# yoshihikosuzuki/ClassPro

Measured on AMD Instinct MI355X. Metric: Mbases/s classified (k=40, 40x HiFi) at 1/2/4/8 MI355X vs CPU -T16, higher is better.
Workload: dtype u16/f64

## Files before the change

### classpro_amd/csrc/capi.hip

```cpp
#include <hip/hip_runtime.h>
#include <stdio.h>
#include <stdlib.h>
#include <string.h>
#include <string>
#include <mutex>
#include <vector>
#include <chrono>
#include <thread>
#include <type_traits>
#include <time.h>
#include "cp_host_setup.h"
#include "kernels.hip"

static thread_local std::string g_err;
static int set_err(int code, const std::string &msg) { g_err = msg; return code; }

#define HIPCHK(call)                                                                       \
  do { hipError_t e_ = (call);                                                             \
       if (e_ != hipSuccess)                                                               \
         return set_err(CP_EHIP,std::string(#call)+": "+hipGetErrorString(e_));            \
     } while (0)
static int launch_status() { HIPCHK(hipGetLastError()); return CP_OK; }

extern "C" const char *cp_last_error(void) { return g_err.c_str(); }
// ... 936 lines not shown
{ if (rlen < 0 || nruns < 0 || K < 1 || (rlen > 0 && !labels) || (nruns > 0 && (!ends || !cls)))
    return set_err(CP_EINVAL,"cp_expand_label_runs: bad argument");
  int pos = K-1 < rlen ? K-1 : rlen;
  memset(labels,'N',(size_t)pos);
  for (int j = 0; j < nruns; j++)
    { const int e = ends[j];
      if (e < pos || e > rlen) return set_err(CP_EINVAL,"cp_expand_label_runs: runs out of order or beyond the read");
      memset(labels+pos,(int)cls[j],(size_t)(e-pos));
      pos = e;
    }
  if (pos != rlen) return set_err(CP_EINVAL,"cp_expand_label_runs: the runs do not cover the read");
  return CP_OK;
}

extern "C" int cp_seq_context(const char *d_seq, const int64_t *d_seq_off, int nreads, int64_t total_bases,
                              uint8_t *d_lctx, uint8_t *d_rctx, void *stream)
{ if (!d_seq || !d_seq_off || !d_lctx || !d_rctx || nreads < 0)
    return set_err(CP_EINVAL,"cp_seq_context: bad argument");
  (void)total_bases;
  if (nreads == 0) return CP_OK;
  hipLaunchKernelGGL(k_seq_context,dim3(nreads),dim3(256),0,(hipStream_t)stream,d_seq,d_seq_off,nreads,d_lctx,d_rctx);
  return launch_status();
}

#ifdef CP_BOUNDS
extern "C" int cp_debug_bounds(unsigned long long *out4)
{ HIPCHK(hipDeviceSynchronize());
  HIPCHK(hipMemcpyFromSymbol(out4,HIP_SYMBOL(g_bounds),sizeof(unsigned long long)*4));
  unsigned long long z[4] = { 0, 0, 0, 0 };
  HIPCHK(hipMemcpyToSymbol(HIP_SYMBOL(g_bounds),z,sizeof(z)));
  return CP_OK;
}
#endif

#if defined(CP_SEED_DEBUG) || defined(CP_SEED_DEBUG_TAKES)
extern "C" int cp_debug_seed_set(int read)
{ HIPCHK(hipMemcpyToSymbol(HIP_SYMBOL(g_seed_dbg_read),&read,sizeof(int))); return CP_OK; }
extern "C" int cp_debug_seed_get(int *out4, int *recs)
{ HIPCHK(hipDeviceSynchronize());
  HIPCHK(hipMemcpyFromSymbol(out4,HIP_SYMBOL(g_seed_dbg_n),16));
  HIPCHK(hipMemcpyFromSymbol(recs,HIP_SYMBOL(g_seed_dbg),8192*16));
  return CP_OK;
}
#endif
#if defined(CP_SEED_PROF) || defined(CP_PROF_WALK)
static int prof_read(unsigned long long *out, const void *sym, size_t n, bool reset = true)
{ static const unsigned long long z[12] = {0};
  HIPCHK(hipMemcpyFromSymbol(out,sym,n*sizeof(unsigned long long)));
  if (reset) HIPCHK(hipMemcpyToSymbol(sym,z,n*sizeof(unsigned long long)));
  return CP_OK;
}
#endif
#ifdef CP_SEED_PROF
extern "C" int cp_debug_seed_prof(unsigned long long *out8)
{ HIPCHK(hipDeviceSynchronize()); return prof_read(out8,HIP_SYMBOL(g_seed_prof),8); }
#endif
extern "C" int cp_debug_task_counts(cp_workspace *ws, int32_t *out, int64_t nreads)
{ if (!ws || !out || nreads < 0 || nreads > ws->nreads || ws->b.fwc.cap < (size_t)nreads*16)
    return set_err(CP_EINVAL,"cp_debug_task_counts: bad arguments");
  HIPCHK(hipDeviceSynchronize());
  if (nreads > 0) HIPCHK(hipMemcpy(out,ws->b.fwc.p,(size_t)nreads*4*sizeof(int32_t),hipMemcpyDeviceToHost));
  return CP_OK;
}
extern "C" int cp_debug_flag_bytes(cp_workspace *ws, int64_t *out2)
{ if (!ws || !out2) return set_err(CP_EINVAL,"cp_debug_flag_bytes: bad arguments");
  HIPCHK(hipDeviceSynchronize());
  const dbuf *arr[2] = { &ws->b.wall, &ws->b.wall_s };
  for (int a = 0; a < 2; a++)
    { std::vector<uint8_t> h(arr[a]->cap);
      if (arr[a]->cap) HIPCHK(hipMemcpy(h.data(),arr[a]->p,arr[a]->cap,hipMemcpyDeviceToHost));
      int64_t n = 0;
      for (uint8_t v : h) n += v != 0;
      out2[a] = n;
    }
  return CP_OK;
}
#ifdef CP_PROF_WALK
extern "C" int cp_debug_live_prof(unsigned long long *out8)
{ HIPCHK(hipDeviceSynchronize()); return prof_read(out8,HIP_SYMBOL(g_live_prof),8); }
extern "C" int cp_debug_emit_prof(unsigned long long *out8)
{ HIPCHK(hipDeviceSynchronize()); return prof_read(out8,HIP_SYMBOL(g_emit_prof),8); }
extern "C" int cp_debug_fw_prof(unsigned long long *out12)
{ HIPCHK(hipDeviceSynchronize()); return prof_read(out12,HIP_SYMBOL(g_fw_prof),12); }
extern "C" int cp_debug_unrel_prof(unsigned long long *out8)
{ HIPCHK(hipDeviceSynchronize()); return prof_read(out8,HIP_SYMBOL(g_unrel_prof),8); }
extern "C" int cp_debug_rel_prof(unsigned long long *out12)
{ HIPCHK(hipDeviceSynchronize()); return prof_read(out12,HIP_SYMBOL(g_rel_prof),12); }
extern "C" int cp_debug_phase_prof(unsigned long long *out36)
{ HIPCHK(hipDeviceSynchronize());
  CHK(prof_read(out36,HIP_SYMBOL(g_phase_max),12));
  CHK(prof_read(out36+12,HIP_SYMBOL(g_phase_sum),12));
  return prof_read(out36+24,HIP_SYMBOL(g_phase_arg),12,false);
}
#endif

#include "kmer_table.hip"

#include "kmer_counts.hip"

#include "kmer_sort.hip"

#include "kmer_lookup.hip"

#include "kmer_hits.hip"

#include "kmer_runs.hip"

#include "kmer_setops.hip"

#include "kmer_cmphist.hip"

#include "kmer_hetpairs.hip"

#include "kmer_unitigs.hip"

#include "kmer_unitig_graph.hip"

#include "kmer_paths.hip"

#include "kmer_prune.hip"

#include "label_tools.hip"
```

### classpro_amd/csrc/kernels.hip

```cpp
#include <hip/hip_runtime.h>
#include <stdint.h>
#include <type_traits>
#include "cp_wall.h"
#include "cp_class.h"
#include "cp_seed.h"

#ifdef CP_BOUNDS
__device__ unsigned long long g_bounds[4];
#endif
#define WAVE 64
#define REL_MAXM 1024
#define UNREL_MAXN 1024
#ifndef REL_SMALL_MAXM
#define REL_SMALL_MAXM 112
#endif
#ifndef UNREL_SMALL_MAXN
#define UNREL_SMALL_MAXN 256
#endif
#define GRP_MAX_PLEN 65535

__device__ __forceinline__ void wave_sync() { __syncthreads(); }
__device__ __forceinline__ void wave_sync_lds()
{ __builtin_amdgcn_fence(__ATOMIC_RELEASE,"wavefront"); __builtin_amdgcn_wave_barrier(); __builtin_amdgcn_fence(__ATOMIC_ACQUIRE,"wavefront"); }

// ... 598 lines not shown
          return true;
        };
      for (int c0 = 0; !done; c0 += WAVE)
        { const int qq = right ? q+1+c0+lane : q-1-c0-lane;
          int pj = 0, fo = 0, fs = 0;
          bool valid = qq >= 0 && qq < F.n;
          if (valid) { pj = F.pos[qq]; valid = right ? (pj < jend) : (pj >= jend); }
          if (valid) { fo = F.fo[qq]; fs = F.fs[qq]; }
          const uint64_t mv = __ballot(valid);
          const uint64_t mw = __ballot(valid && (((fo & CP_W_WALL_O) | (fs & CP_W_WALL_S)) != 0));
          const uint64_t ms = __ballot(valid && (fo & CP_W_WALL_O));
          for (uint64_t t = mw; t; t &= t-1)
            { const int b = __ffsll((long long)t)-1;
              const int jj = __shfl(pj,b), qj = right ? q+1+c0+b : q-1-c0-b;
              if (nx > 0 && !flush_x(jj)) return;
              if (cp_bs_eintvl(ev,0,NS-1,right ? i : jj,right ? jj : i) == -1)
                { const double pe_j = CP_PERR(R,jj,CP_SELF,right ? CP_GAIN : CP_DROP);
                  const double pe = pe_i * pe_j;
                  if (pe >= CP_PE_THRES_FINAL)
                    { if (*midx >= R->ecap) { R->overflow = 1; return; }
                      ev.wave_grow(*midx);
                      if (lane == 0)
                        { cp_eintvl x; x.b = right ? i : jj; x.e = right ? jj : i; x.pe = pe;
                          ev.put(*midx,x);
                          F.fo[q] |= CP_W_PAIRED_M;
                          F.fo[qj] |= CP_W_PAIRED_M;
                        }
                      (*midx)++;
                      if (*midx >= plen) { R->overflow = 8; return; }
                    }
                }
              if ((ms >> b) & 1) { done = true; break; }
            }
          if (mv != ~0ull) break;
        }
      if (nx > 0 && !done && !flush_x(right ? 0x7fffffff : -1)) return;
      if (!done && (right ? plen < jend : jend == 0))
        { const double pe = pe_i * pe_i;
          if (pe >= CP_PE_THRES_FINAL)
            { if (*midx >= R->ecap) { R->overflow = 1; return; }
              ev.wave_grow(*midx);
              if (lane == 0)
                { cp_eintvl x; x.b = right ? i : 0; x.e = right ? plen : i; x.pe = pe;
                  ev.put(*midx,x);
                  F.fo[q] |= CP_W_PAIRED_M;
                }
              (*midx)++;
              if (*midx >= plen) { R->overflow = 8; return; }
            }
        }
      wave_sync();
    }
}

#define CP_PCLS(e,a)   (((uint32_t)(e) << 3) | ((uint32_t)(a) & 7u))
#define CP_PCLS_END(x) ((int)((x) >> 3))
#define CP_PCLS_CLS(x) (((x) & 7u) == 7u ? -1 : (int)((x) & 7u))

struct cp_rrec { int32_t b, e; uint16_t ccb, cce; int32_t idx; double pe; };
static_assert(sizeof(cp_rrec) == 24,"compact reliable-interval record");
struct cp_ivA { int32_t b, e; uint16_t cb, ce, ccb, cce; };
struct cp_ivB { double pe, peo_b, peo_e; };
struct cp_ivC { uint8_t is_rel; int8_t asgn; };
static_assert(sizeof(cp_ivA) == 16 && sizeof(cp_ivB) == 24 && sizeof(cp_ivC) == 2,"interval records as arrays");
struct cp_soa { cp_ivA *a; cp_ivB *b; cp_ivC *c; };
__device__ __forceinline__ void cp_soa_put(const cp_soa &S, int64_t at, const cp_intvl &I)
{ cp_ivA a; a.b = I.b; a.e = I.e; a.cb = I.cb; a.ce = I.ce; a.ccb = I.ccb; a.cce = I.cce;
  cp_ivB b; b.pe = I.pe; b.peo_b = I.peo_b; b.peo_e = I.peo_e;
  cp_ivC c; c.is_rel = I.is_rel; c.asgn = I.asgn;
  S.a[at] = a; S.b[at] = b; S.c[at] = c;
}
__device__ __forceinline__ cp_intvl cp_soa_get(const cp_soa &S, int64_t at)
{ const cp_ivA a = S.a[at]; const cp_ivB b = S.b[at]; const cp_ivC c = S.c[at];
  cp_intvl I;
  memset(&I,0,sizeof(I));
  I.b = a.b; I.e = a.e; I.cb = a.cb; I.ce = a.ce; I.ccb = a.ccb; I.cce = a.cce;
  I.is_rel = c.is_rel; I.asgn = c.asgn; I.pe = b.pe; I.peo_b = b.peo_b; I.peo_e = b.peo_e;
  return I;
}

#ifdef CP_PROF_WALK
__device__ unsigned long long g_phase_max[12], g_phase_sum[12], g_phase_arg[12];
__device__ unsigned long long g_live_prof[8];
__device__ unsigned long long g_unrel_prof[8];
__device__ unsigned long long g_emit_prof[8];
__device__ unsigned long long g_fw_prof[12];
#define EM_LT0() unsigned long long em_t = wall_clock64()
#define EM_LT(k) do { unsigned long long t_ = wall_clock64(); if (lane == 0) atomicAdd(&g_fw_prof[4+(k)],t_-em_t); em_t = wall_clock64(); } while (0)
#define PH_STAMP(k) do { if (lane == 0) { unsigned long long t_ = wall_clock64(); unsigned long long d_ = t_-ph_t; ph_t = t_; \
      atomicAdd(&g_phase_sum[k],d_); unsigned long long o_ = atomicMax(&g_phase_max[k],d_); if (d_ > o_) g_phase_arg[k] = ((unsigned long long)r << 32) | (unsigned)n_c; } } while (0)
#elif defined(CP_STOP_AT)
#define PH_STAMP(k) do { if ((k) == CP_STOP_AT) { PH_STOP_EXTRA; return; } } while (0)
#else
#define PH_STAMP(k) ((void)0)
#endif
#ifndef EM_LT0
#define EM_LT0() ((void)0)
#define EM_LT(k) ((void)0)
#endif
#define PH_STOP_EXTRA

struct task_res { double own_pe, lc_v, hc_pe; int lc_j, hc, pos, kc; };
#define TR_E(hc)     (((hc) >> 3) & 1)
#define TR_WTYPE(hc) (((hc) >> 4) & 1)
static_assert(sizeof(task_res) == 40,"three doubles and four ints, no padding");
static_assert(CP_DROP == 0 && CP_GAIN == 1 && CP_SELF == 0 && CP_OTHERS == 1,"one bit each in task_res::hc");
static_assert(CP_LC_REJECT <= 3,"lc_kind takes two bits of task_res::hc");
struct task_stage { double own_pe, lc_v, hc_pe; int lc_j, hc; };

#define FW_SEQ_WIN    32
#define FW_SEQ_STRIDE 36
struct cp_seq_lwin
  { CP_SEQ_T g; CP_LDS_PTR(const char) w; int lo, len;
    __device__ __forceinline__ char operator[](int p) const
    { const unsigned d = (unsigned)(p-lo); return d < (unsigned)len ? w[d] : g[p]; }
  };
__device__ __forceinline__ int cp_seq_dirword(const cp_seq_lwin &sq, int rlen, int pos, int dir, uint64_t *D)
{ (void)rlen;
  const int d = (dir > 0 ? pos : pos-7)-sq.lo;
  if (d < 0 || d+8 > sq.len) return 0;
  CP_LDS_PTR(const uint32_t) rw = (CP_LDS_PTR(const uint32_t))(sq.w+(d & ~3));
  const uint32_t x0 = rw[0], x1 = rw[1], x2 = rw[2];
  const uint32_t sh = (uint32_t)(d & 3)*8;
  const uint32_t lo = __builtin_amdgcn_alignbit(x1,x0,sh), hi = __builtin_amdgcn_alignbit(x2,x1,sh);
  const uint64_t x = (uint64_t)lo | ((uint64_t)hi << 32);
  *D = dir > 0 ? x : __builtin_bswap64(x);
  return 8;
}
struct __attribute__((packed, aligned(1))) cp_u8x16 { uint32_t v[4]; };
struct __attribute__((packed, aligned(1))) cp_u8x4 { uint32_t v; };
struct cp_seq_rwin
  { CP_SEQ_T g;
    uint64_t wl, wh;
    int lo, len;
    __device__ __forceinline__ char operator[](int p) const
    { const unsigned d = (unsigned)(p-lo);
      if (d < (unsigned)len)
        { const uint64_t x = (d < 8) ? wl : wh;
          return (char)(x >> ((d & 7)*8));
        }
      return g[p];
    }
  };
__device__ __forceinline__ int cp_seq_dirword(const cp_seq_rwin &sq, int rlen, int pos, int dir, uint64_t *D)
{ (void)rlen;
  const int d = (dir > 0 ? pos : pos-7)-sq.lo;
  if (sq.len != 16 || d < 0 || d > 8) return 0;
  const uint64_t x = d == 0 ? sq.wl : d == 8 ? sq.wh : (sq.wl >> (8*d)) | (sq.wh << (64-8*d));
  *D = dir > 0 ? x : __builtin_bswap64(x);
  return 8;
}
struct cp_seq_rsrc { CP_SEQ_T g; };
__device__ __forceinline__ cp_seq_rwin cp_seq_window(const cp_seq_rsrc &src, int pos, int rlen, int dir)
{ cp_seq_rwin sq;
  int lo = dir > 0 ? pos-7 : pos-11;
  if (lo > rlen-16) lo = rlen-16;
  if (lo < 0) lo = 0;
  sq.g = src.g; sq.lo = lo; sq.len = 0; sq.wl = sq.wh = 0;
  if (rlen-lo >= 16)
    { const cp_u8x16 x = *reinterpret_cast<const cp_u8x16 *>(CP_SPAN(src.g,lo,16));
      sq.wl = (uint64_t)x.v[0] | ((uint64_t)x.v[1] << 32);
      sq.wh = (uint64_t)x.v[2] | ((uint64_t)x.v[3] << 32);
      sq.len = 16;
    }
  return sq;
}

// ... 1632 lines not shown
__device__ __forceinline__ void quad_cov_sums(const Rv &rv, const int8_t *asgn, int M, int ld, int cls, int &lsum, int &csum)
{ int ls = 0, cs = 0;
  for (int i = ld; i < M; i += 4)
    if (cls < 0 || asgn[i] == cls)
      { const cp_riv I = rv(i);
        const int l = I.e-I.b;
        ls += l;
        cs += (I.ccb+I.cce)*l/2;
      }
  lsum = quad_isum(ls); csum = quad_isum(cs);
}
__device__ __forceinline__ int quad_count(const int8_t *asgn, int M, int ld, int cls)
{ int n = 0;
  for (int i = ld; i < M; i += 4) n += (asgn[i] == cls);
  return quad_isum(n);
}
__device__ __forceinline__ void quad_first_last(const int8_t *asgn, int M, int ld, int cls, int &first, int &last)
{ int f = M, l = -1;
  for (int i = ld; i < M; i += 4)
    if (asgn[i] == cls) { if (f == M) f = i; l = i; }
  f = quad_imin(f); last = quad_imax(l);
  first = (f == M) ? -1 : f;
}
template <class Rv>
__device__ bool rel_post1_quad(const cp_dev_params *P, const Rv &rv, int M, int F, const int8_t *asgn, int *COV, int ld)
{ const int *G = P->cov;
  if (quad_count(asgn,M,ld,CP_HAPLO)) return false;
  int first_d, last_d;
  quad_first_last(asgn,M,ld,CP_DIPLO,first_d,last_d);
  const int seed = F ? first_d : last_d;
  if (seed < 0) return false;
  int lsum, csum;
  quad_cov_sums(rv,asgn,M,ld,CP_DIPLO,lsum,csum);
  const double mean_dcov = (double)csum/lsum;
  if (!(mean_dcov < G[CP_DIPLO])) return false;
  const cp_riv S = rv(seed);
  COV[CP_HAPLO] = F ? S.ccb : S.cce;
  COV[CP_DIPLO] = (COV[CP_HAPLO]+G[CP_HAPLO]) & 0xffff;
  return true;
}
template <class Rv>
__device__ double rel_post2_quad(const cp_dev_params *P, const Rv &rv, int M, int8_t *asgn, bool rerun, int ld)
{ const int *G = P->cov;
  int lsum, csum;
  if (rerun && quad_count(asgn,M,ld,CP_HAPLO) == 0)
    { quad_cov_sums(rv,asgn,M,ld,CP_DIPLO,lsum,csum);
      const double mean_dcov = (double)csum/lsum;
      if (fabs(mean_dcov-G[CP_HAPLO]) <= fabs(mean_dcov-G[CP_DIPLO]))
        for (int i = ld; i < M; i += 4)
          if (asgn[i] == CP_DIPLO) asgn[i] = CP_HAPLO;
    }
  int n = quad_count(asgn,M,ld,CP_HAPLO);
  if (n == M)
    { quad_cov_sums(rv,asgn,M,ld,-1,lsum,csum);
      const double mean_hcov = (double)csum/lsum;
      if (fabs(mean_hcov-G[CP_HAPLO]) >= fabs(mean_hcov-G[CP_DIPLO]))
        { for (int i = ld; i < M; i += 4) asgn[i] = CP_DIPLO;
          n = 0;
        }
    }
  if (n >= M * 0.7)
    { quad_cov_sums(rv,asgn,M,ld,CP_HAPLO,lsum,csum);
      const double mean_hcov = (double)csum/lsum;
      if (fabs(mean_hcov-G[CP_HAPLO]) >= fabs(mean_hcov-G[CP_DIPLO]))
        for (int i = ld; i < M; i += 4)
          { if (asgn[i] == CP_HAPLO)      asgn[i] = CP_DIPLO;
            else if (asgn[i] == CP_DIPLO) asgn[i] = CP_REPEAT;
          }
    }
  int first_d, last_d, first_h, last_h;
  quad_first_last(asgn,M,ld,CP_DIPLO,first_d,last_d);
  quad_first_last(asgn,M,ld,CP_HAPLO,first_h,last_h);
  if (!(first_d >= 0 && first_h >= 0))
    return 1.;
  return ((double)rv(first_d).ccb/rv(first_h).ccb)/((double)rv(last_d).cce/rv(last_h).cce);
}

#ifndef REL_SMALL_G
#define REL_SMALL_G 8
#endif
#ifndef UNREL_SMALL_G
#define UNREL_SMALL_G 2
#endif
#ifndef UNREL_BIG_G
#define UNREL_BIG_G 1
#endif
#ifndef REL_EXTRA_ATTR
#define REL_EXTRA_ATTR
#endif
#ifndef REL_SMALL_WPB
#define REL_SMALL_WPB 2
#endif
#ifndef REL_WAVES_PER_EU
#define REL_WAVES_PER_EU 3
#endif

template <int MINM, int MAXM, int G, int WPB, int COMPACT = 0>
__global__ void __launch_bounds__(WAVE*WPB) __attribute__((amdgpu_waves_per_eu(G == 8 ? REL_WAVES_PER_EU : 2))) REL_EXTRA_ATTR
k_classify_rel_grp(const cp_dev_params *__restrict__ P, const int64_t *__restrict__ prof_off, int nreads,
                   cp_intvl *__restrict__ intvl_all, cp_intvl *__restrict__ rintvl_all, const int32_t *__restrict__ relmap_all,
                   const int64_t *__restrict__ ioff, const int32_t *__restrict__ nrel,
                   int8_t *__restrict__ asgn_all, int64_t totalI, const int32_t *__restrict__ perm,
                   const cp_rrec *__restrict__ rrec_all, cp_soa soa)
{
  __shared__ rel_grp_lds<MAXM,G> Sw[WPB];
  __shared__ rel_libm_lds T;
  for (int k = threadIdx.x; k < 256; k += WAVE*WPB)
    { T.exp_tab[k] = cp_libm::exp_tab[k]; T.log_tab[k] = cp_libm::log_tab[k]; }
  __syncthreads();
  const int wv = threadIdx.x/WAVE;
  rel_grp_lds<MAXM,G> &S = Sw[wv];
  constexpr int L = WAVE/G;
  const int lane = lane_id();
  const int g = lane/L, ql = lane%L;
  for (int blk = blockIdx.x*WPB+wv; blk*G < nreads; blk += gridDim.x*WPB)
  {
  const int slot = blk*G+g;
  const int r = (slot < nreads) ? perm[slot] : nreads;
  int M = (r < nreads) ? nrel[r] : 0;
  const int rr = (r < nreads) ? r : 0;
  const int plen = (int)(prof_off[rr+1]-prof_off[rr]);
  if (MINM > 0 && __ballot(M > MINM || (r < nreads && plen > GRP_MAX_PLEN)) == 0) break;
  if (M <= MINM || M > MAXM || plen > GRP_MAX_PLEN) M = 0;
  if (__ballot(M > 0) == 0) continue;
  const int64_t o = ioff[rr];
  cp_intvl *rintvl = rintvl_all+o;
  const cp_rrec *rrec = COMPACT ? rrec_all+o : nullptr;
  rel_rec<COMPACT> rec; rec.rrec = rrec; rec.rintvl = rintvl;
  if constexpr (G != 8)
  {
  if (COMPACT)
    for (int k = ql; k < M; k += L)
      { const cp_rrec q = rrec[k];
        S.b[g][k] = (uint16_t)q.b; S.e[g][k] = (uint16_t)q.e; S.ccb[g][k] = q.ccb; S.cce[g][k] = q.cce;
      }
  else
    for (int k = ql; k < M; k += L)
      { S.b[g][k] = (uint16_t)rintvl[k].b; S.e[g][k] = (uint16_t)rintvl[k].e;
        S.ccb[g][k] = rintvl[k].ccb; S.cce[g][k] = rintvl[k].cce;
      }
  grp_sync<WPB>();
  }

  constexpr int LD = REL_LD(G);
  const int d = (ql / LD) & 1, F = (d == 0);
  const int leadlane = g*L+d*LD;
  const bool lead = (M > 0) && (ql < 2*LD) && ((ql % LD) == 0);
  int COV[4] = { P->cov[0], P->cov[1], P->cov[2], P->cov[3] };
#ifdef CP_PROF_WALK
  const unsigned long long rp_g0 = wall_clock64();
#endif
  typename std::conditional<G == 8,rel_rec<COMPACT>,rel_grp_rv<MAXM,G>>::type rv;
  if constexpr (G == 8) rv = rec;
  else { rv.S = &S; rv.g = g; }
  rel_grp_pass<MAXM,G,WPB>(P,S,T,rec,M,plen,M > 0,COV);

  RP_DECL(7);
  int rerun = 0;
  if constexpr (G == 8)
    { if (M > 0) rerun = rel_post1_quad(P,rv,M,F,S.asgn(g,d),COV,ql % LD) ? 1 : 0; }
  else
  if (lead)
    rerun = cp_rel_post1(P,rv,M,F,S.asgn(g,d),COV) ? 1 : 0;
  rerun = __shfl(rerun,leadlane);
  COV[CP_HAPLO] = __shfl(COV[CP_HAPLO],leadlane);
  COV[CP_DIPLO] = __shfl(COV[CP_DIPLO],leadlane);
// ... 33 lines not shown
      for (int i = 0; i < M; i++)
        if (fw[i] != bw[i]) { eq = false; break; }
      if (!eq)
        { bool pre = (fw[0] == 1);
          if (pre)
            { int i = 0;
              while (i < M && fw[i]) i++;
              while (i < M) { if (fw[i]) { pre = false; break; } i++; }
            }
          if (!pre)
            { bool suf = (fw[M-1] == 1);
              if (suf)
                { int i = M-2;
                  while (i >= 0 && fw[i]) i--;
                  while (i >= 0) { if (fw[i]) { suf = false; break; } i--; }
                }
              if (suf) take_bw = 1;
              else if (!(fabs(hf-1.) <= fabs(hb-1.))) take_bw = 1;
            }
        }
    }
  take_bw = __shfl(take_bw,g*L);
  RP_STAMP(2);
  cp_intvl *intvl = intvl_all+o;
  const int32_t *relmap = relmap_all+o;
  int8_t *gfw = asgn_all+o, *gbw = asgn_all+totalI+o;
  if (COMPACT)
    for (int i = ql; i < M; i += L)
      { const int8_t a = take_bw ? S.asgn(g,1)[i] : S.asgn(g,0)[i];
        if (soa.c) soa.c[o+rrec[i].idx].asgn = a; else intvl[rrec[i].idx].asgn = a;
      }
  else
  for (int i = ql; i < M; i += L)
    { int8_t f = S.asgn(g,0)[i], w = S.asgn(g,1)[i];
      int8_t a = take_bw ? w : f;
      gfw[i] = f; gbw[i] = w;
      rintvl[i].asgn = a;
      intvl[relmap[i]].asgn = a;
      if (soa.c) soa.c[o+relmap[i]].asgn = a;
    }
  grp_sync<WPB>();
  RP_STAMP(6);
#ifdef CP_PROF_WALK
  rp_acc[3] = wall_clock64()-rp_g0; rp_acc[4] = 1;
#endif
  RP_FLUSH(G == 8,5,11,5);
  }
}

template <int MAXN, int G>
struct unrel_grp_lds
  { static_assert(MAXN % 64 == 0,"the reliable-interval bitsets are whole 64-bit words"); uint16_t b[G][MAXN], e[G][MAXN], cb[G][MAXN], ce[G][MAXN], ccb[G][MAXN], cce[G][MAXN];
    int8_t   asgn[G][MAXN];
    uint8_t  isrel[G][MAXN];
    typedef typename std::conditional<(MAXN > 256),uint32_t,uint16_t>::type ord_t;
    ord_t    ord[G][MAXN];
    uint16_t key[G][MAXN+4];
    uint64_t rel[G][2][MAXN/64];
    uint64_t need[G][MAXN/64];
  };

__device__ __forceinline__ int bits_left(const uint64_t *bits, int idx)
{ int w = idx >> 6;
  uint64_t m = bits[w] & ((1ull << (idx & 63))-1);
  while (true)
    { if (m) return (w << 6)+63-__clzll((long long)m);
      if (--w < 0) return -1;
      m = bits[w];
    }
}
__device__ __forceinline__ int bits_right(const uint64_t *bits, int idx, int nwords)
{ int w = idx >> 6;
  uint64_t m = bits[w] & ~((2ull << (idx & 63))-1);
  while (true)
    { if (m) return (w << 6)+__ffsll((long long)m)-1;
      if (++w >= nwords) return -1;
      m = bits[w];
    }
}

#ifndef UNREL_WAVES_PER_EU
#define UNREL_WAVES_PER_EU 4
#endif
template <int MINN, int MAXN, int G, int COMPACT = 0>
__global__ void __launch_bounds__(WAVE) __attribute__((amdgpu_waves_per_eu(UNREL_WAVES_PER_EU)))
k_classify_unrel_grp(const cp_dev_params *__restrict__ P, int nreads, cp_intvl *__restrict__ intvl_all,
                     const int64_t *__restrict__ ioff, const int32_t *__restrict__ nintvl,
                     const int32_t *__restrict__ perm, const int64_t *__restrict__ prof_off, uint32_t *__restrict__ pcls_all,
                     cp_soa soa, int full_sweep2)
{
  __shared__ unrel_grp_lds<MAXN,G> S;
  constexpr int L = WAVE/G;
  static_assert(L >= 8 && (L % 8) == 0, "8 role lanes per read");
  const int lane = lane_id();
  const int g = lane/L, ql = lane%L, gbase = g*L;
  constexpr int K = L/8;
  const int sub = ql >> 3, role = ql & 7, sbase = gbase+sub*8;
  const int s2 = (role >> 2) & 1, side = (role >> 1) & 1, kind = role & 1;
  const int s = s2 ? CP_DIPLO : CP_HAPLO;
  const double *const skel = P->skel, *const uerr = P->uerr, *const logfact = P->logfact;
  const int skel_kmax = P->skel_kmax, uerr_max = P->uerr_max;
  const long long skel_cdmax = P->skel_cdmax;
  const int covE = P->cov[CP_ERROR], REP = P->cov[CP_REPEAT], covH = P->cov[CP_HAPLO], covD = P->cov[CP_DIPLO];
  const double llE = cp_poisson_loglambda(P,covE), llH = cp_poisson_loglambda(P,covH), llD = cp_poisson_loglambda(P,covD);
  const double dr_ratio = P->dr_ratio, r_lp = P->r_lp, r_l1mp = P->r_l1mp;
  for (int blk = blockIdx.x; blk*G < nreads; blk += gridDim.x)
  {
#ifdef CP_PROF_WALK
  const unsigned long long ur_t0 = wall_clock64();
#endif
  const int slot = blk*G+g;
  const int r = (slot < nreads) ? perm[slot] : nreads;
  int N = (r < nreads) ? nintvl[r] : 0;
  const int rr = (r < nreads) ? r : 0;
  const bool too_long = prof_off[rr+1]-prof_off[rr] > GRP_MAX_PLEN;
  if (MINN > 0 && __ballot(N > MINN || (r < nreads && too_long)) == 0) break;
  const int64_t io = ioff[rr];
  cp_intvl *intvl = intvl_all+io;
  if (N <= MINN || N > MAXN || too_long) N = 0;
  if (__ballot(N > 0) == 0) continue;
#ifdef CP_PROF_WALK
  unsigned long long ur_commit = 0, ur_pre = 0, ur_use = 0, ur_load = 0, ur_sort = 0, ur_t = wall_clock64();
#define UR_STAMP(acc) do { const unsigned long long t_ = wall_clock64(); acc += t_-ur_t; ur_t = t_; } while (0)
#else
#define UR_STAMP(acc) ((void)0)
#endif
  const int nwords = (N+63) >> 6;
  int maxN = N;
  for (int o = 32; o > 0; o >>= 1)
    { int x = __shfl_xor(maxN,o); maxN = x > maxN ? x : maxN; }

  for (int k = ql; k < MAXN/64; k += L)
    { S.rel[g][0][k] = 0; S.rel[g][1][k] = 0; S.need[g][k] = ~0ull; }
  wave_sync();
  for (int base = 0; base < maxN; base += L)
    { const int k = base+ql;
      bool h = false, dd = false;
      if (k < N && COMPACT)
        { const cp_ivA A = soa.a[io+k]; const cp_ivC Cc = soa.c[io+k];
          S.b[g][k] = (uint16_t)A.b; S.e[g][k] = (uint16_t)A.e;
          S.cb[g][k] = A.cb; S.ce[g][k] = A.ce; S.ccb[g][k] = A.ccb; S.cce[g][k] = A.cce;
          S.asgn[g][k] = Cc.asgn; S.isrel[g][k] = Cc.is_rel;
          h  = Cc.is_rel && Cc.asgn == CP_HAPLO;
          dd = Cc.is_rel && Cc.asgn == CP_DIPLO;
        }
      else if (k < N)
        { cp_intvl I = intvl[k];
          if (soa.c) I.asgn = soa.c[io+k].asgn;
          S.b[g][k] = (uint16_t)I.b; S.e[g][k] = (uint16_t)I.e;
          S.cb[g][k] = I.cb; S.ce[g][k] = I.ce; S.ccb[g][k] = I.ccb; S.cce[g][k] = I.cce;
          S.asgn[g][k] = I.asgn; S.isrel[g][k] = I.is_rel;
          h  = I.is_rel && I.asgn == CP_HAPLO;
          dd = I.is_rel && I.asgn == CP_DIPLO;
        }
      const uint64_t mh = __ballot(h) >> gbase, md = __ballot(dd) >> gbase;
      if (ql == 0 && base < N)
        { const uint64_t lm = (L == 64) ? ~0ull : ((1ull << L)-1);
          S.rel[g][0][base >> 6] |= (mh & lm) << (base & 63);
          S.rel[g][1][base >> 6] |= (md & lm) << (base & 63);
        }
    }
  wave_sync();
  UR_STAMP(ur_load);
  constexpr int RSH = (MAXN > 256) ? 16 : 8;
  int nnf = 0;
  for (int base = 0; base < maxN; base += L)
    { const int i = base+ql;
      const bool keep = i < N && !(S.isrel[g][i] && (S.asgn[g][i] == CP_HAPLO || S.asgn[g][i] == CP_DIPLO));
      const uint64_t lm = (L == 64) ? ~0ull : ((1ull << L)-1);
      const uint64_t mk = (__ballot(keep) >> gbase) & lm;
      if (keep) S.ord[g][nnf+__popcll(mk & ((1ull << ql)-1))] = (typename unrel_grp_lds<MAXN,G>::ord_t)i;
      nnf += __popcll(mk);
    }
  wave_sync();
  for (int j = ql; j < ((nnf+3) & ~3); j += L)
    { uint16_t key = 0xffff;
      if (j < nnf) { const int k = S.ord[g][j]; key = S.cb[g][k] < S.ce[g][k] ? S.cb[g][k] : S.ce[g][k]; }
      S.key[g][j] = key;
    }
  wave_sync();
  for (int j = ql; j < nnf; j += L)
    { const unsigned key = S.key[g][j];
      int rank = 0;
      for (int m = 0; m < nnf; m += 4)
        { const uint2 q = *reinterpret_cast<const uint2 *>(&S.key[g][m]);
          const unsigned k0 = q.x & 0xffffu, k1 = q.x >> 16, k2 = q.y & 0xffffu, k3 = q.y >> 16;
          rank += (k0 < key || (k0 == key && m   < j)) ? 1 : 0;
          rank += (k1 < key || (k1 == key && m+1 < j)) ? 1 : 0;
          rank += (k2 < key || (k2 == key && m+2 < j)) ? 1 : 0;
          rank += (k3 < key || (k3 == key && m+3 < j)) ? 1 : 0;
        }
      S.ord[g][j] = (typename unrel_grp_lds<MAXN,G>::ord_t)((unsigned)S.ord[g][j] | ((unsigned)rank << RSH));
    }
  wave_sync();
  for (int j = ql; j < nnf; j += L)
    { const unsigned v = S.ord[g][j];
      S.key[g][v >> RSH] = (uint16_t)(v & ((1u << RSH)-1));
    }
#define S_ORD(p) ((int)S.key[g][p])
  nnf = __shfl(nnf,gbase);
  int maxNF = nnf;
  for (int o = 32; o > 0; o >>= 1)
    { int x = __shfl_xor(maxNF,o); maxNF = x > maxNF ? x : maxNF; }
  wave_sync();

  const uint64_t glm = (L == 64) ? ~0ull : ((1ull << L)-1);
  int pass = 0, it = 0;
  bool done = (N == 0) || (nnf == 0);
#ifdef CP_PROF_WALK
  int prof_rounds[2] = { 0, 0 };
#endif
  UR_STAMP(ur_sort);
  while (__ballot(!done) != 0)
      { int mypos = it+sub;
        int cover = (it+K < nnf) ? it+K : nnf;
        if (pass == 1)
          { const int p = it+ql;
            bool dirty = false;
            if (!done && p < nnf)
              { const int k = S_ORD(p);
                dirty = full_sweep2 || ((S.need[g][k >> 6] >> (k & 63)) & 1);
              }
            const uint64_t m = (__ballot(dirty) >> gbase) & glm;
            uint64_t t = m;
            for (int j = 0; j < sub; j++) t &= t-1;
            mypos = t ? it+__ffsll((long long)t)-1 : nnf;
            uint64_t t2 = m;
#pragma unroll
            for (int j = 0; j < K; j++) t2 &= t2-1;
            cover = t2 ? it+__ffsll((long long)t2)-1 : ((it+L < nnf) ? it+L : nnf);
          }
        const bool act = !done && mypos < nnf;
        bool on = act;
        int idx = 0;
        if (act)
          idx = S_ORD(pass == 0 ? nnf-1-mypos : mypos);
        int snew = -1;
        int Icb = 0, Ice = 0, lH = -1, rH = -1, lD = -1, rD = -1;
        if (on)
          { Icb = S.cb[g][idx]; Ice = S.ce[g][idx];
            if ((Icb > Ice ? Icb : Ice) >= REP)
              { snew = CP_REPEAT;
                on = false;
              }
            else
              { lH = bits_left(S.rel[g][0],idx); rH = bits_right(S.rel[g][0],idx,nwords);
                lD = bits_left(S.rel[g][1],idx); rD = bits_right(S.rel[g][1],idx,nwords);
              }
          }
        UR_STAMP(ur_pre);
        bool do_sf = false, do_bin = false, in_tab = false, r_in = false;
        int oa = 0, ob = 0, oc = 0;
        int kb = 0, ke = 0, nl = 0, nr = 0;
        double er = -INFINITY, val = -INFINITY, pe = 0., lfb = 0., lfe = 0., lfnl = 0., lfdl = 0., lfnr = 0., lfdr = 0.;
        if (on)
          { const double *const rec = COMPACT ? &soa.b[io+idx].pe : &intvl[idx].pe;
            const double *const rec_er = side ? (COMPACT ? &soa.b[io+idx].peo_e : &intvl[idx].peo_e)
                                              : (COMPACT ? &soa.b[io+idx].peo_b : &intvl[idx].peo_b);
            const int nb = side ? idx+1 : idx-1;
            if (kind == 0 && nb >= 0 && nb < N && S.asgn[g][nb] == (int8_t)s) er = *rec_er;
            pe = *rec;
            kb = cp_check_cnt(Icb); ke = cp_check_cnt(Ice);
            lfb = logfact[kb]; lfe = logfact[ke];
            { int dcov_l, dcov_r;
              if (lD == -1 && rD == -1) dcov_l = dcov_r = covD;
              else if (lD == -1)        dcov_l = dcov_r = S.cb[g][rD];
              else if (rD == -1)        dcov_l = dcov_r = S.ce[g][lD];
              else                      { dcov_l = S.ce[g][lD]; dcov_r = S.cb[g][rD]; }
              const int rcov_l = (uint16_t)(dr_ratio*dcov_l);
              const int rcov_r = (uint16_t)(dr_ratio*dcov_r);
              r_in = !(Icb >= rcov_l || Ice >= rcov_r);
              if (r_in)
                { nl = cp_check_cnt(rcov_l); nr = cp_check_cnt(rcov_r);
                  lfnl = logfact[nl]; lfdl = logfact[nl-kb]; lfnr = logfact[nr]; lfdr = logfact[nr-ke];
                }
            }
            const double *at = nullptr;
            const int Ib = S.b[g][idx], Ie = S.e[g][idx];
            const int l_rel = s2 ? lD : lH, r_rel = s2 ? rD : rH;
            if (kind == 0)
              { int tb = 0, te = 0, tcb = 0, tce = 0, tcov = 0;
                if (side == 0 && l_rel != -1)
                  { do_sf = true; tb = S.e[g][l_rel]-1; te = Ib; tcb = S.cce[g][l_rel]; tce = Icb; tcov = tcb; }
                if (side == 1 && r_rel != -1)
                  { do_sf = true; tb = Ie-1; te = S.b[g][r_rel]; tcb = Ice; tce = S.ccb[g][r_rel]; tcov = tce; }
                if (do_sf)
                  { oa = tce-tcb; ob = tcov & 0xffff; oc = te-tb < 0 ? tb-te : te-tb;
                    at = cp_logp_trans_at(skel,skel_kmax,skel_cdmax,oc,tcb,tce,ob);
                  }
              }
            else
              { const int x = side ? Ie-1 : Ib;
                const int c = side ? Ice : Icb;
                int ll = l_rel, rr = r_rel, e1 = -1;
                for (int rep = 0; rep < 2 && e1 < 0; rep++)
                  { if (ll != -1 && rr != -1)
                      e1 = (int)(uint16_t)cp_linear_interpolation(x,S.e[g][ll]-1,S.cce[g][ll],S.b[g][rr],S.ccb[g][rr]);
                    else if (ll != -1) e1 = S.cce[g][ll];
                    else if (rr != -1) e1 = S.ccb[g][rr];
                    if (e1 < 0)
                      { if (rep == 0) { ll = s2 ? lH : lD; rr = s2 ? rH : rD; }
                        else e1 = -2;
                      }
                    else if (rep == 1)
                      e1 = (e1 > 0) ? (((s == CP_HAPLO) ? e1/2 : e1*2) & 0xffff) : -2;
                  }
                const int est = (e1 >= 0) ? e1 : (s2 ? covD : covH);
                do_bin = est >= c;
                if (do_bin)
                  { oa = est; ob = c;
                    at = cp_logp_uerr_at(uerr,uerr_max,est,c);
                  }
              }
            in_tab = at != nullptr;
            if (in_tab) val = *at;
          }
        if (do_sf && !in_tab)
          val = cp_logp_trans_calc(P,oa,(double)ob*oc);
        if (do_bin && !in_tab)
          val = cp_logp_uerr_calc(P,oa,ob);
        if (on)
          { if (kind == 0)
              val = (er > val) ? er : val;
            double v1 = __shfl_down(val,1);
            double sidev = (val > v1) ? val : v1;
            double vr = __shfl_down(sidev,2);
            double logp_l = sidev, logp_r = vr;
            if (logp_l == -INFINITY && logp_r == -INFINITY)
              { logp_l = cp_logp_poisson_vals(kb,s2 ? llD : llH,s2 ? covD : covH,lfb);
                logp_r = cp_logp_poisson_vals(ke,s2 ? llD : llH,s2 ? covD : covH,lfe);
              }
            else if (logp_l == -INFINITY) logp_l = logp_r;
            else if (logp_r == -INFINITY) logp_r = logp_l;
            const double logp_s = logp_l+logp_r;
            const double vH = __shfl(logp_s,sbase), vD = __shfl(logp_s,sbase+4);
            const double po = cp_logp_poisson_vals(kb,llE,covE,lfb)+cp_logp_poisson_vals(ke,llE,covE,lfe)+CP_E_PO_BASE;
            const double vE = (pe > po) ? pe : po;
            double vR = CP_R_LOGP;
            if (r_in)
              vR = cp_logp_binom_vals(lfnl,lfb,lfdl,kb,nl,r_lp,r_l1mp)+cp_logp_binom_vals(lfnr,lfe,lfdr,ke,nr,r_lp,r_l1mp);
            double logpmax = -INFINITY;
            if (logpmax < vE) { logpmax = vE; snew = CP_ERROR; }
            if (logpmax < vR) { logpmax = vR; snew = CP_REPEAT; }
            if (logpmax < vH) { logpmax = vH; snew = CP_HAPLO; }
            if (logpmax < vD) { logpmax = vD; snew = CP_DIPLO; }
          }
        wave_sync();
        UR_STAMP(ur_use);
        const bool lead = role == 0, upd = act && snew >= 0;
        int old = 0;
        bool hd = false, setc = false;
        if (lead && upd)
          { old = S.asgn[g][idx];
            const bool ohd = old == CP_HAPLO || old == CP_DIPLO, nhd = snew == CP_HAPLO || snew == CP_DIPLO;
            hd = old != snew && (ohd || nhd);
            setc = hd && S.isrel[g][idx];
          }
        const uint64_t m_hd = __ballot(hd), m_setc = __ballot(setc);
        const int osl = gbase+8*(role & (K-1));
        const int oidx = __shfl(idx,osl);
        const bool cl = role < sub && (((m_setc >> osl) & 1) || (((m_hd >> osl) & 1) && (oidx == idx-1 || oidx == idx+1)));
        constexpr uint64_t LEADS = 0x0101010101010101ull & ((L == 64) ? ~0ull : ((1ull << L)-1));
        const uint64_t clm = (__ballot(cl) >> gbase) & glm;
        const uint64_t cb = ((clm | ((clm & 0x7f7f7f7f7f7f7f7full)+0x7f7f7f7f7f7f7f7full)) >> 7) & LEADS;
        const uint64_t ub = (__ballot(lead && upd) >> gbase) & glm;
        const uint64_t stop = (~ub & LEADS) | cb;
        const int js = stop ? __ffsll((long long)stop)-1 : L;
        const uint64_t hb = ((m_hd >> gbase) & glm) & (js < 64 ? (1ull << js)-1 : ~0ull);
        const bool hstop = pass == 1 && hb != 0;
        const int jh = hstop ? __ffsll((long long)hb)-1 : 0;
        const bool cstop = !hstop && js < L && ((ub >> js) & 1);
        const int spos = __shfl(mypos,gbase+(hstop ? jh : cstop ? js : 0));
        const int newit = hstop ? spos+1 : cstop ? spos : cover;
        const bool cm = lead && upd && ql < (hstop ? jh+1 : js);
        unsigned long long *const need = reinterpret_cast<unsigned long long *>(S.need[g]);
        if (cm) atomicAnd(&need[idx >> 6],~(1ull << (idx & 63)));
        if (cm && hd)
          { if (idx > 0)   atomicOr(&need[(idx-1) >> 6],1ull << ((idx-1) & 63));
            if (idx+1 < N) atomicOr(&need[(idx+1) >> 6],1ull << ((idx+1) & 63));
          }
        if (cm && old != snew) S.asgn[g][idx] = (int8_t)snew;
        if (cm && setc)
          { const uint64_t bit = 1ull << (idx & 63);
            for (int q = 0; q < 2; q++)
              { const int sq = q ? CP_DIPLO : CP_HAPLO;
                if (old != sq && snew != sq) continue;
                int lo = bits_left(S.rel[g][q],idx), hi = bits_right(S.rel[g][q],idx,nwords);
                if (lo < 0) lo = 0;
                if (hi < 0) hi = N-1;
                for (int w = lo >> 6; w <= (hi >> 6); w++)
                  { const uint64_t ml = (w == (lo >> 6)) ? (~0ull << (lo & 63)) : ~0ull;
                    const uint64_t mh = (w == (hi >> 6)) ? (~0ull >> (63-(hi & 63))) : ~0ull;
                    atomicOr(&need[w],ml & mh);
                  }
                if (old == sq) S.rel[g][q][idx >> 6] &= ~bit; else S.rel[g][q][idx >> 6] |= bit;
              }
          }
        UR_STAMP(ur_commit);
#ifdef CP_PROF_WALK
        if (!done) prof_rounds[pass]++;
#endif
        if (!done)
          { it = newit;
            if (it >= nnf) { it = 0; pass++; if (pass == 2) done = true; }
          }
        wave_sync();
      }
#ifdef CP_PROF_WALK
  if (ql == 0 && N > 0 && MINN == 0)
    { atomicAdd(&g_phase_sum[9],(unsigned long long)prof_rounds[0]); atomicAdd(&g_phase_max[9],(unsigned long long)prof_rounds[1]);
      atomicAdd(&g_phase_sum[10],(unsigned long long)nnf); atomicAdd(&g_phase_sum[11],1ull); }
  if (lane == 0 && MINN == 0)
    { atomicAdd(&g_unrel_prof[0],ur_commit); atomicAdd(&g_unrel_prof[1],ur_pre); atomicAdd(&g_unrel_prof[4],ur_use);
      atomicAdd(&g_unrel_prof[5],ur_load); atomicAdd(&g_unrel_prof[6],ur_sort);
      atomicAdd(&g_unrel_prof[2],wall_clock64()-ur_t0); atomicAdd(&g_unrel_prof[3],1ull); }
#endif
#undef UR_STAMP
  if (pcls_all)
    for (int k = ql; k < N; k += L)
      pcls_all[io+k] = CP_PCLS((int)S.e[g][k],S.asgn[g][k]);
  else
    for (int k = ql; k < N; k += L)
      intvl[k].asgn = S.asgn[g][k];
  wave_sync();
  }
}

#define PAINT_MAX 512
#define PAINT_TILE 2048
__device__ __forceinline__ int wave_scan_add(int v)
{ v += __builtin_amdgcn_update_dpp(0,v,0x111,0xf,0xf,false);
  v += __builtin_amdgcn_update_dpp(0,v,0x112,0xf,0xf,false);
  v += __builtin_amdgcn_update_dpp(0,v,0x114,0xf,0xf,false);
  v += __builtin_amdgcn_update_dpp(0,v,0x118,0xf,0xf,false);
  v += __builtin_amdgcn_update_dpp(0,v,0x142,0xa,0xf,false);
  v += __builtin_amdgcn_update_dpp(0,v,0x143,0xc,0xf,false);
  return v;
}
__device__ __forceinline__ unsigned cp_label_char(int a)
{ return (a == CP_ERROR) ? 'E' : (a == CP_REPEAT) ? 'R' : (a == CP_HAPLO) ? 'H' : (a == CP_DIPLO) ? 'D' : '?'; }

__global__ void __launch_bounds__(WAVE)
k_paint_labels(const cp_dev_params *__restrict__ P, const int64_t *__restrict__ seq_off, int nreads,
               const cp_intvl *__restrict__ intvl_all, const int64_t *__restrict__ ioff,
               const int32_t *__restrict__ nintvl, char *__restrict__ labels, const uint32_t *__restrict__ pcls_all)
{ const int r = blockIdx.x;
  if (r >= nreads) return;
  const int lane = lane_id();
  const int K = P->K;
  const uint32_t *pcls = pcls_all ? pcls_all+ioff[r] : nullptr;
  char *lab = labels+seq_off[r];
  const int rlen = (int)(seq_off[r+1]-seq_off[r]);
  const cp_intvl *intvl = intvl_all+ioff[r];
  const int N = nintvl[r];
  __shared__ int s_end[PAINT_MAX];
  __shared__ uint8_t s_chr[PAINT_MAX];
  __shared__ __attribute__((aligned(16))) uint32_t s_cnt[PAINT_TILE/2];
  if (N+1 <= PAINT_MAX)
    { if (lane == 0) { s_end[0] = K-1 < rlen ? K-1 : rlen; s_chr[0] = 'N'; }
      if (pcls)
        for (int k = lane; k < N; k += WAVE)
          { const uint32_t x = pcls[k]; s_end[k+1] = CP_PCLS_END(x)+(K-1); s_chr[k+1] = (uint8_t)cp_label_char(CP_PCLS_CLS(x)); }
      else
      for (int k = lane; k < N; k += WAVE)
        { s_end[k+1] = intvl[k].e+(K-1); s_chr[k+1] = (uint8_t)cp_label_char(intvl[k].asgn); }
      wave_sync();
      const int M = N+1;
      auto find = [&](int q) -> int
        { int lo = 0, hi = M-1;
          while (lo < hi) { const int m = (lo+hi) >> 1; if (s_end[m] > q) hi = m; else lo = m+1; }
          return lo;
        };
      const int head = (int)((16-((uintptr_t)lab & 15)) & 15);
      const int h = head < rlen ? head : rlen;
      if (lane < h) lab[lane] = (char)s_chr[find(lane)];
      const int npiece = (rlen-h) >> 4;
      uint4 *dst = reinterpret_cast<uint4 *>(lab+h);
      int carry = 0;
      for (int p0 = 0; p0 < npiece; p0 += PAINT_TILE)
        { const int np = npiece-p0 < PAINT_TILE ? npiece-p0 : PAINT_TILE;
          for (int j = lane; 4*j < ((np+WAVE-1) & ~(WAVE-1)); j += WAVE)
            reinterpret_cast<uint2 *>(s_cnt)[j] = make_uint2(0u,0u);
          wave_sync();
          for (int k = lane; k < M; k += WAVE)
            { const int e = s_end[k];
              const int p = (e <= h ? 0 : (e-h+15) >> 4)-p0;
              if (p >= 0 && p < np) atomicAdd(&s_cnt[p >> 1],1u << (16*(p & 1)));
            }
          wave_sync();
          for (int base = 0; base < np; base += WAVE)
            { const int pc = p0+base+lane;
              const int inc = wave_scan_add((int)reinterpret_cast<const uint16_t *>(s_cnt)[base+lane]);
              int k = carry+inc;
              carry += wave_of_last(inc);
// ... 383 lines not shown
```

Baseline: 390,500.

## Use 4 lanes per unreliable-interval slot and widen pass-2 dirty scan window

The unreliable-interval classification kernel now defaults to 4 role lanes per slot instead of 8. Each lane computes both the self/flanking transition term and the binomial error term, so twice as many intervals are evaluated per wave round. The pass-2 dirty-interval search now scans a window of two wave-widths, so more dirty intervals can be picked up per round. The trade is more per-lane work and registers, plus extra shuffle loops for the conflict check. Profiling counters for the large-N variant are also added.

```diff
diff --git a/classpro_amd/csrc/capi.hip b/classpro_amd/csrc/capi.hip
--- a/classpro_amd/csrc/capi.hip
+++ b/classpro_amd/csrc/capi.hip
@@ -1042,8 +1042,8 @@
 { HIPCHK(hipDeviceSynchronize()); return prof_read(out8,HIP_SYMBOL(g_emit_prof),8); }
 extern "C" int cp_debug_fw_prof(unsigned long long *out12)
 { HIPCHK(hipDeviceSynchronize()); return prof_read(out12,HIP_SYMBOL(g_fw_prof),12); }
-extern "C" int cp_debug_unrel_prof(unsigned long long *out8)
-{ HIPCHK(hipDeviceSynchronize()); return prof_read(out8,HIP_SYMBOL(g_unrel_prof),8); }
+extern "C" int cp_debug_unrel_prof(unsigned long long *out12)
+{ HIPCHK(hipDeviceSynchronize()); return prof_read(out12,HIP_SYMBOL(g_unrel_prof),12); }
 extern "C" int cp_debug_rel_prof(unsigned long long *out12)
 { HIPCHK(hipDeviceSynchronize()); return prof_read(out12,HIP_SYMBOL(g_rel_prof),12); }
 extern "C" int cp_debug_phase_prof(unsigned long long *out36)
diff --git a/classpro_amd/csrc/kernels.hip b/classpro_amd/csrc/kernels.hip
--- a/classpro_amd/csrc/kernels.hip
+++ b/classpro_amd/csrc/kernels.hip
@@ -704,7 +704,7 @@
 #ifdef CP_PROF_WALK
 __device__ unsigned long long g_phase_max[12], g_phase_sum[12], g_phase_arg[12];
 __device__ unsigned long long g_live_prof[8];
-__device__ unsigned long long g_unrel_prof[8];
+__device__ unsigned long long g_unrel_prof[12];
 __device__ unsigned long long g_emit_prof[8];
 __device__ unsigned long long g_fw_prof[12];
 #define EM_LT0() unsigned long long em_t = wall_clock64()
@@ -2503,6 +2503,12 @@
 #ifndef UNREL_SMALL_G
 #define UNREL_SMALL_G 2
 #endif
+#ifndef UNREL_LPS
+#define UNREL_LPS 4
+#endif
+#ifndef UNREL_SWEEP2_WIN
+#define UNREL_SWEEP2_WIN 2
+#endif
 #ifndef UNREL_BIG_G
 #define UNREL_BIG_G 1
 #endif
@@ -2702,7 +2708,7 @@
 #ifndef UNREL_WAVES_PER_EU
 #define UNREL_WAVES_PER_EU 4
 #endif
-template <int MINN, int MAXN, int G, int COMPACT = 0>
+template <int MINN, int MAXN, int G, int COMPACT = 0, int LPS = UNREL_LPS>
 __global__ void __launch_bounds__(WAVE) __attribute__((amdgpu_waves_per_eu(UNREL_WAVES_PER_EU)))
 k_classify_unrel_grp(const cp_dev_params *__restrict__ P, int nreads, cp_intvl *__restrict__ intvl_all,
                      const int64_t *__restrict__ ioff, const int32_t *__restrict__ nintvl,
@@ -2711,12 +2717,14 @@
 {
   __shared__ unrel_grp_lds<MAXN,G> S;
   constexpr int L = WAVE/G;
-  static_assert(L >= 8 && (L % 8) == 0, "8 role lanes per read");
+  static_assert((LPS == 4 || LPS == 8) && L >= LPS, "4 or 8 role lanes per slot");
   const int lane = lane_id();
   const int g = lane/L, ql = lane%L, gbase = g*L;
-  constexpr int K = L/8;
-  const int sub = ql >> 3, role = ql & 7, sbase = gbase+sub*8;
-  const int s2 = (role >> 2) & 1, side = (role >> 1) & 1, kind = role & 1;
+  constexpr int K = L/LPS;
+  constexpr bool BOTH = LPS == 4;
+  const int sub = ql/LPS, role = ql%LPS, sbase = gbase+sub*LPS;
+  const int cs = BOTH ? role : role >> 1, kind = BOTH ? 0 : role & 1;
+  const int s2 = (cs >> 1) & 1, side = cs & 1;
   const int s = s2 ? CP_DIPLO : CP_HAPLO;
   const double *const skel = P->skel, *const uerr = P->uerr, *const logfact = P->logfact;
   const int skel_kmax = P->skel_kmax, uerr_max = P->uerr_max;
@@ -2835,20 +2843,27 @@
       { int mypos = it+sub;
         int cover = (it+K < nnf) ? it+K : nnf;
         if (pass == 1)
-          { const int p = it+ql;
-            bool dirty = false;
-            if (!done && p < nnf)
-              { const int k = S_ORD(p);
-                dirty = full_sweep2 || ((S.need[g][k >> 6] >> (k & 63)) & 1);
+          { uint64_t m[2] = { 0, 0 };
+#pragma unroll
+            for (int h = 0; h < UNREL_SWEEP2_WIN; h++)
+              { const int p = it+h*L+ql;
+                bool dirty = false;
+                if (!done && p < nnf)
+                  { const int k = S_ORD(p);
+                    dirty = full_sweep2 || ((S.need[g][k >> 6] >> (k & 63)) & 1);
+                  }
+                m[h] = (__ballot(dirty) >> gbase) & glm;
               }
-            const uint64_t m = (__ballot(dirty) >> gbase) & glm;
-            uint64_t t = m;
-            for (int j = 0; j < sub; j++) t &= t-1;
-            mypos = t ? it+__ffsll((long long)t)-1 : nnf;
-            uint64_t t2 = m;
-#pragma unroll
-            for (int j = 0; j < K; j++) t2 &= t2-1;
-            cover = t2 ? it+__ffsll((long long)t2)-1 : ((it+L < nnf) ? it+L : nnf);
+            const int c0 = __popcll(m[0]);
+            auto nth = [&](int n) -> int
+              { const bool hi = n >= c0;
+                uint64_t t = hi ? m[1] : m[0];
+                for (int j = hi ? n-c0 : n; j > 0; j--) t &= t-1;
+                return t ? (hi ? L : 0)+__ffsll((long long)t)-1 : -1;
+              };
+            const int mine = nth(sub), next = nth(K);
+            mypos = mine >= 0 ? it+mine : nnf;
+            cover = next >= 0 ? it+next : ((it+UNREL_SWEEP2_WIN*L < nnf) ? it+UNREL_SWEEP2_WIN*L : nnf);
           }
         const bool act = !done && mypos < nnf;
         bool on = act;
@@ -2869,10 +2884,11 @@
               }
           }
         UR_STAMP(ur_pre);
-        bool do_sf = false, do_bin = false, in_tab = false, r_in = false;
+        bool do_sf = false, do_bin = false, sf_tab = false, bin_tab = false, r_in = false;
         int oa = 0, ob = 0, oc = 0;
+        int ua = 0, uc = 0;
         int kb = 0, ke = 0, nl = 0, nr = 0;
-        double er = -INFINITY, val = -INFINITY, pe = 0., lfb = 0., lfe = 0., lfnl = 0., lfdl = 0., lfnr = 0., lfdr = 0.;
+        double er = -INFINITY, vsf = -INFINITY, vbin = -INFINITY, pe = 0., lfb = 0., lfe = 0., lfnl = 0., lfdl = 0., lfnr = 0., lfdr = 0.;
         if (on)
           { const double *const rec = COMPACT ? &soa.b[io+idx].pe : &intvl[idx].pe;
             const double *const rec_er = side ? (COMPACT ? &soa.b[io+idx].peo_e : &intvl[idx].peo_e)
@@ -2895,10 +2911,10 @@
                   lfnl = logfact[nl]; lfdl = logfact[nl-kb]; lfnr = logfact[nr]; lfdr = logfact[nr-ke];
                 }
             }
-            const double *at = nullptr;
+            const double *at_sf = nullptr, *at_bin = nullptr;
             const int Ib = S.b[g][idx], Ie = S.e[g][idx];
             const int l_rel = s2 ? lD : lH, r_rel = s2 ? rD : rH;
-            if (kind == 0)
+            if (BOTH || kind == 0)
               { int tb = 0, te = 0, tcb = 0, tce = 0, tcov = 0;
                 if (side == 0 && l_rel != -1)
                   { do_sf = true; tb = S.e[g][l_rel]-1; te = Ib; tcb = S.cce[g][l_rel]; tce = Icb; tcov = tcb; }
@@ -2906,10 +2922,10 @@
                   { do_sf = true; tb = Ie-1; te = S.b[g][r_rel]; tcb = Ice; tce = S.ccb[g][r_rel]; tcov = tce; }
                 if (do_sf)
                   { oa = tce-tcb; ob = tcov & 0xffff; oc = te-tb < 0 ? tb-te : te-tb;
-                    at = cp_logp_trans_at(skel,skel_kmax,skel_cdmax,oc,tcb,tce,ob);
+                    at_sf = cp_logp_trans_at(skel,skel_kmax,skel_cdmax,oc,tcb,tce,ob);
                   }
               }
-            else
+            if (BOTH || kind == 1)
               { const int x = side ? Ie-1 : Ib;
                 const int c = side ? Ice : Icb;
                 int ll = l_rel, rr = r_rel, e1 = -1;
@@ -2928,23 +2944,30 @@
                 const int est = (e1 >= 0) ? e1 : (s2 ? covD : covH);
                 do_bin = est >= c;
                 if (do_bin)
-                  { oa = est; ob = c;
-                    at = cp_logp_uerr_at(uerr,uerr_max,est,c);
+                  { ua = est; uc = c;
+                    at_bin = cp_logp_uerr_at(uerr,uerr_max,est,c);
                   }
               }
-            in_tab = at != nullptr;
-            if (in_tab) val = *at;
+            sf_tab = at_sf != nullptr; bin_tab = at_bin != nullptr;
+            if (sf_tab)  vsf = *at_sf;
+            if (bin_tab) vbin = *at_bin;
           }
-        if (do_sf && !in_tab)
-          val = cp_logp_trans_calc(P,oa,(double)ob*oc);
-        if (do_bin && !in_tab)
-          val = cp_logp_uerr_calc(P,oa,ob);
+        if (do_sf && !sf_tab)
+          vsf = cp_logp_trans_calc(P,oa,(double)ob*oc);
+        if (do_bin && !bin_tab)
+          vbin = cp_logp_uerr_calc(P,ua,uc);
         if (on)
-          { if (kind == 0)
-              val = (er > val) ? er : val;
-            double v1 = __shfl_down(val,1);
-            double sidev = (val > v1) ? val : v1;
-            double vr = __shfl_down(sidev,2);
+          { double sidev;
+            if constexpr (BOTH)
+              { const double a = (er > vsf) ? er : vsf;
+                sidev = (a > vbin) ? a : vbin;
+              }
+            else
+              { const double val = (kind == 0) ? ((er > vsf) ? er : vsf) : vbin;
+                const double v1 = __shfl_down(val,1);
+                sidev = (val > v1) ? val : v1;
+              }
+            double vr = __shfl_down(sidev,LPS/4);
             double logp_l = sidev, logp_r = vr;
             if (logp_l == -INFINITY && logp_r == -INFINITY)
               { logp_l = cp_logp_poisson_vals(kb,s2 ? llD : llH,s2 ? covD : covH,lfb);
@@ -2953,7 +2976,7 @@
             else if (logp_l == -INFINITY) logp_l = logp_r;
             else if (logp_r == -INFINITY) logp_r = logp_l;
             const double logp_s = logp_l+logp_r;
-            const double vH = __shfl(logp_s,sbase), vD = __shfl(logp_s,sbase+4);
+            const double vH = __shfl(logp_s,sbase), vD = __shfl(logp_s,sbase+LPS/2);
             const double po = cp_logp_poisson_vals(kb,llE,covE,lfb)+cp_logp_poisson_vals(ke,llE,covE,lfe)+CP_E_PO_BASE;
             const double vE = (pe > po) ? pe : po;
             double vR = CP_R_LOGP;
@@ -2977,12 +3000,18 @@
             setc = hd && S.isrel[g][idx];
           }
         const uint64_t m_hd = __ballot(hd), m_setc = __ballot(setc);
-        const int osl = gbase+8*(role & (K-1));
-        const int oidx = __shfl(idx,osl);
-        const bool cl = role < sub && (((m_setc >> osl) & 1) || (((m_hd >> osl) & 1) && (oidx == idx-1 || oidx == idx+1)));
-        constexpr uint64_t LEADS = 0x0101010101010101ull & ((L == 64) ? ~0ull : ((1ull << L)-1));
+        bool cl = false;
+#pragma unroll
+        for (int c = 0; c < (K+LPS-1)/LPS; c++)
+          { const int o = role+c*LPS;
+            const int osl = gbase+LPS*(o & (K-1));
+            const int oidx = __shfl(idx,osl);
+            cl |= o < sub && (((m_setc >> osl) & 1) || (((m_hd >> osl) & 1) && (oidx == idx-1 || oidx == idx+1)));
+          }
+        constexpr uint64_t LEADS = (LPS == 8 ? 0x0101010101010101ull : 0x1111111111111111ull) & ((L == 64) ? ~0ull : ((1ull << L)-1));
+        constexpr uint64_t LOWS  = (LPS == 8 ? 0x7f7f7f7f7f7f7f7full : 0x7777777777777777ull);
         const uint64_t clm = (__ballot(cl) >> gbase) & glm;
-        const uint64_t cb = ((clm | ((clm & 0x7f7f7f7f7f7f7f7full)+0x7f7f7f7f7f7f7f7full)) >> 7) & LEADS;
+        const uint64_t cb = ((clm | ((clm & LOWS)+LOWS)) >> (LPS-1)) & LEADS;
         const uint64_t ub = (__ballot(lead && upd) >> gbase) & glm;
         const uint64_t stop = (~ub & LEADS) | cb;
         const int js = stop ? __ffsll((long long)stop)-1 : L;
@@ -3030,6 +3059,9 @@
   if (ql == 0 && N > 0 && MINN == 0)
     { atomicAdd(&g_phase_sum[9],(unsigned long long)prof_rounds[0]); atomicAdd(&g_phase_max[9],(unsigned long long)prof_rounds[1]);
       atomicAdd(&g_phase_sum[10],(unsigned long long)nnf); atomicAdd(&g_phase_sum[11],1ull); }
+  if (ql == 0 && N > 0 && MINN > 0)
+    { atomicAdd(&g_unrel_prof[8],(unsigned long long)prof_rounds[0]); atomicAdd(&g_unrel_prof[9],(unsigned long long)prof_rounds[1]);
+      atomicAdd(&g_unrel_prof[10],(unsigned long long)nnf); atomicAdd(&g_unrel_prof[11],1ull); }
   if (lane == 0 && MINN == 0)
     { atomicAdd(&g_unrel_prof[0],ur_commit); atomicAdd(&g_unrel_prof[1],ur_pre); atomicAdd(&g_unrel_prof[4],ur_use);
       atomicAdd(&g_unrel_prof[5],ur_load); atomicAdd(&g_unrel_prof[6],ur_sort);
```

New measurement: 403,100, median of 6. +3.2%, better.
